# ISU-PAAL/DeepDFA

Hardware: AMD Instinct MI355X
Metric: train_graphs_per_sec (higher is better)
Workload: dtype bf16; 1 GPU; model=DeepDFA-FlowGNN-GGNN(n_steps=5,D=128), global_batch=256, avg_nodes_per_graph=45, parallelism=dp1

## Files before the change

csrc/bindings.hip:

```cpp

#include <torch/extension.h>

#include <hip/hip_runtime.h>
#include <hip/hip_bf16.h>
#include <c10/hip/HIPStream.h>
#include <c10/util/accumulate.h>

#include <climits>

template <typename T>
void launch_embed4_fwd(const T*, const long*, T*, int, int, hipStream_t);
template <typename T, typename TO>
void launch_embed4_fwd2(const T*, const long*, TO*, int, int, hipStream_t);
template <typename T>
void launch_embed4_bwd(const T*, const long*, float*, long, int, hipStream_t);
template <typename T>
void launch_spmm_sum(const int*, const int*, const T*, T*, int, int, hipStream_t);
template <typename T>
void launch_gru_gates_fwd(const T*, const T*, const T*, T*, T*, T*, T*, long, int, hipStream_t);
template <typename T>
void launch_gru_gates_bwd(const T*, const T*, const T*, const T*, const T*, const T*, T*, T*, T*,
                          long, int, hipStream_t);
template <typename T>
void launch_attn_pool_fwd(const T*, const T*, const int*, T*, float*, int, int, hipStream_t);
template <typename T>
void launch_attn_pool_bwd(const T*, const T*, const float*, const int*, T*, T*, float*, int, int,
                          hipStream_t);
void launch_segment_max(const float*, const int*, float*, int, hipStream_t);
template <typename T>
void launch_gru_gates2_fwd(const T*, const T*, T*, T*, T*, T*, T*, long, int, hipStream_t);
template <typename T>
void launch_gru_gates2_bwd(const T*, const T*, const T*, const T*, const T*, const T*, T*, T*,
                           long, int, hipStream_t);
template <typename T>
void launch_colsum(const T*, float*, int, int, hipStream_t);
template <typename T>
void launch_spmm_sum_strided(const int*, const int*, const T*, T*, int, int, long,
                             hipStream_t);
void launch_gemm_bias2(const __hip_bfloat16*, const __hip_bfloat16*, const __hip_bfloat16*,
                       const __hip_bfloat16*, const __hip_bfloat16*, long,
                       const __hip_bfloat16*, long, __hip_bfloat16*, int, int, int, int,
                       hipStream_t);
void launch_gemm_bias(const __hip_bfloat16*, const __hip_bfloat16*, const __hip_bfloat16*,
                      const __hip_bfloat16*, const __hip_bfloat16*, __hip_bfloat16*, int, int,
                      int, int, hipStream_t);
void launch_wgrad(const __hip_bfloat16*, const __hip_bfloat16*, const __hip_bfloat16*, float*,
                  float*, int, int, int, int, hipStream_t, float* = nullptr,
                  float* = nullptr, float* = nullptr, float* = nullptr);
template <typename T>
void launch_layernorm_fwd(const T*, const float*, const float*, T*, float*, float*, long, int,
                          float, hipStream_t);
template <typename T>
void launch_layernorm_bwd(const T*, const T*, const float*, const float*, const float*, T*, long,
                          int, hipStream_t);
template <typename T>
void launch_layernorm_wgrad(const T*, const T*, const float*, const float*, float*, float*, long,
                            int, hipStream_t);
template <typename T>
void launch_bias_gelu_fwd(const T*, const float*, T*, long, int, hipStream_t);
template <typename T>
void launch_bias_gelu_bwd(const T*, const T*, const float*, T*, long, int, hipStream_t);
template <typename T>
void launch_softmax_mask_fwd(const T*, const int*, T*, T*, long, int, int, float, float,
                             unsigned long long, int, int, hipStream_t);
template <typename T>
// ... 264 lines not shown
  CHECK_GPU(B);
  const int K = A.size(0), M = A.size(1), C = B.size(1);
  TORCH_CHECK(B.size(0) == K && M % 64 == 0 && C % 8 == 0);
  const bool acc = out_opt.has_value();
  auto out = acc_or_zeros(out_opt, {M, C}, A.options(), "wgrad");
  if (M % 128 == 0 && C % 128 == 0) {
    launch_wgrad2(ptr<bf16_t>(A), ptr<bf16_t>(B), out.data_ptr<float>(), nullptr,
                  K, M, C, acc ? 1 : 0, cur_stream());
    return out;
  }
  launch_wgrad(ptr<bf16_t>(A), ptr<bf16_t>(B), nullptr, out.data_ptr<float>(), nullptr,
               K, M, C, C, cur_stream());
  return out;
}

void launch_pack_gru_weights(const float*, const float*, const float*, const float*,
                             const float*, const float*, int, __hip_bfloat16*,
                             __hip_bfloat16*, __hip_bfloat16*, __hip_bfloat16*,
                             __hip_bfloat16*, __hip_bfloat16*, __hip_bfloat16*,
                             __hip_bfloat16*, hipStream_t);
void launch_gemm_gru(const __hip_bfloat16*, const __hip_bfloat16*, const __hip_bfloat16*,
                     const __hip_bfloat16*, const __hip_bfloat16*, __hip_bfloat16*,
                     __hip_bfloat16*, __hip_bfloat16*, __hip_bfloat16*, __hip_bfloat16*,
                     int, int, int, int, hipStream_t);

void pack_gru_weights(at::Tensor W_e, at::Tensor b_e, at::Tensor W_ih, at::Tensor W_hh,
                      at::Tensor b_ih, at::Tensor b_hh, at::Tensor w_e16, at::Tensor b_e16,
                      at::Tensor Wcat, at::Tensor WcatT, at::Tensor b_cat, at::Tensor W_eT,
                      at::Tensor Wcat_perm, at::Tensor b_perm) {
  CHECK_GPU(W_e);
  const int H = W_e.size(0);
  TORCH_CHECK(W_e.scalar_type() == at::kFloat && W_ih.scalar_type() == at::kFloat,
              "pack_gru_weights reads fp32 master weights");
  TORCH_CHECK(Wcat.size(0) == 4 * H && Wcat.size(1) == 2 * H);
  launch_pack_gru_weights(W_e.data_ptr<float>(), b_e.data_ptr<float>(),
                          W_ih.data_ptr<float>(), W_hh.data_ptr<float>(),
                          b_ih.data_ptr<float>(), b_hh.data_ptr<float>(), H,
                          mptr<bf16_t>(w_e16), mptr<bf16_t>(b_e16), mptr<bf16_t>(Wcat),
                          mptr<bf16_t>(WcatT), mptr<bf16_t>(b_cat), mptr<bf16_t>(W_eT),
                          mptr<bf16_t>(Wcat_perm), mptr<bf16_t>(b_perm),
                          cur_stream());
}

std::vector<at::Tensor> ggnn_fused_fwd(at::Tensor indptr, at::Tensor indices, at::Tensor x,
                                       at::Tensor W_e, at::Tensor b_e, at::Tensor Wcat_perm,
                                       at::Tensor b_perm, long n_steps) {
  CHECK_GPU(x);
  TORCH_CHECK(x.scalar_type() == at::kBFloat16, "fused GGNN path is bf16");
  const long N = x.size(0);
  const long H = x.size(1);
  TORCH_CHECK(H % 64 == 0 && (4 * H) % 128 == 0, "H must suit the MFMA tile");
  TORCH_CHECK(Wcat_perm.size(0) == 4 * H && Wcat_perm.size(1) == 2 * H &&
              b_perm.numel() == 4 * H,
              "Wcat_perm/b_perm must be prebuilt (ops/flowgnn.py cache)");
  auto stream = cur_stream();
  const long S = n_steps;
  auto opts = x.options();
  auto HH = at::empty({S + 1, N, H}, opts);
  HH.select(0, 0).copy_(x);
  auto M = at::empty({S, N, H}, opts);
  auto R = at::empty({S, N, H}, opts);
  auto Z = at::empty({S, N, H}, opts);
  auto Nn = at::empty({S, N, H}, opts);
  auto HN = at::empty({S, N, H}, opts);
  auto wh = at::empty({N, H}, opts);
  const long NH = N * H;
  for (long s = 0; s < S; ++s) {
    const bf16_t* h = ptr<bf16_t>(HH) + s * NH;
    launch_gemm_bias(h, nullptr, ptr<bf16_t>(W_e), ptr<bf16_t>(b_e), nullptr, mptr<bf16_t>(wh),
                     N, H, H, H, stream);
    bf16_t* m = mptr<bf16_t>(M) + s * NH;
    launch_spmm_sum<bf16_t>(indptr.data_ptr<int>(), indices.data_ptr<int>(), ptr<bf16_t>(wh), m,
                            N, H, stream);
    launch_gemm_gru(m, h, ptr<bf16_t>(Wcat_perm), ptr<bf16_t>(b_perm), h,
                    mptr<bf16_t>(HH) + (s + 1) * NH, mptr<bf16_t>(R) + s * NH,
                    mptr<bf16_t>(Z) + s * NH, mptr<bf16_t>(Nn) + s * NH,
                    mptr<bf16_t>(HN) + s * NH, N, 2 * H, H, H, stream);
  }
  auto h_final = HH.select(0, S);
  return {h_final, HH, M, R, Z, Nn, HN};
}

std::vector<at::Tensor> ggnn_fused_bwd(at::Tensor grad_out, at::Tensor t_indptr,
                                       at::Tensor t_indices, at::Tensor x, at::Tensor W_eT,
                                       at::Tensor WcatT, at::Tensor HH,
                                       at::Tensor M, at::Tensor R, at::Tensor Z, at::Tensor Nn,
                                       at::Tensor HN, long n_steps,
                                       c10::optional<at::Tensor> out_we,
                                       c10::optional<at::Tensor> out_be,
                                       c10::optional<std::vector<at::Tensor>> gru_outs) {
  const long N = x.size(0);
  const long H = x.size(1);
  const long S = n_steps;
  const long NH = N * H;
  auto stream = cur_stream();
  TORCH_CHECK(WcatT.size(0) == 2 * H && WcatT.size(1) == 4 * H && W_eT.size(0) == H,
              "WcatT/W_eT must be prebuilt (ops/flowgnn.py cache)");
  auto opts = x.options();
  auto Ggicat = at::empty({S, N, 4 * H}, opts);
  auto Gwh = at::empty({S, N, H}, opts);
  auto grad_h = grad_out.contiguous().clone();
  auto grad_hd = at::empty({N, H}, opts);
  auto grad_A = at::empty({N, 2 * H}, opts);
  for (long s = S - 1; s >= 0; --s) {
    const bf16_t* h_in = ptr<bf16_t>(HH) + s * NH;
    auto ggic = Ggicat.select(0, s);
    auto gwh = Gwh.select(0, s);
    launch_gru_gates2_bwd<bf16_t>(ptr<bf16_t>(grad_h), h_in, ptr<bf16_t>(R) + s * NH,
                                  ptr<bf16_t>(Z) + s * NH, ptr<bf16_t>(Nn) + s * NH,
                                  ptr<bf16_t>(HN) + s * NH, mptr<bf16_t>(ggic),
                                  mptr<bf16_t>(grad_hd), NH, H, stream);
    launch_gemm_bias(ptr<bf16_t>(ggic), nullptr, ptr<bf16_t>(WcatT), nullptr, nullptr,
                     mptr<bf16_t>(grad_A), N, 4 * H, 4 * H, 2 * H, stream);
    launch_spmm_sum_strided<bf16_t>(t_indptr.data_ptr<int>(), t_indices.data_ptr<int>(),
                                    ptr<bf16_t>(grad_A), mptr<bf16_t>(gwh), N, H,
                                    2 * H, stream);
    launch_gemm_bias2(ptr<bf16_t>(gwh), nullptr, ptr<bf16_t>(W_eT), nullptr,
                      ptr<bf16_t>(grad_hd), H, ptr<bf16_t>(grad_A) + H, 2 * H,
                      mptr<bf16_t>(grad_h), N, H, H, H, stream);
  }
  auto A_g = Ggicat.view({S * N, 4 * H});
  const bool gru_direct = gru_outs.has_value();
  at::Tensor gWcat, cs4;
  if (gru_direct) {
    TORCH_CHECK(gru_outs->size() == 4, "gru_outs = [gW_ih, gW_hh, gb_ih, gb_hh]");
    for (auto& t : *gru_outs)
      TORCH_CHECK(t.is_cuda() && t.scalar_type() == at::kFloat && t.is_contiguous());
    TORCH_CHECK((*gru_outs)[0].numel() == 3 * H * H &&
                (*gru_outs)[1].numel() == 3 * H * H &&
                (*gru_outs)[2].numel() == 3 * H && (*gru_outs)[3].numel() == 3 * H);
  } else {
    gWcat = at::zeros({4 * H, 2 * H}, opts.dtype(at::kFloat));
    cs4 = at::zeros({4 * H}, opts.dtype(at::kFloat));
  }
  if (gru_direct)
    launch_wgrad(ptr<bf16_t>(A_g), ptr<bf16_t>(M), ptr<bf16_t>(HH), nullptr, nullptr,
                 S * N, 4 * H, 2 * H, H, stream, (*gru_outs)[0].data_ptr<float>(),
                 (*gru_outs)[1].data_ptr<float>(), (*gru_outs)[2].data_ptr<float>(),
                 (*gru_outs)[3].data_ptr<float>());
  else
    launch_wgrad(ptr<bf16_t>(A_g), ptr<bf16_t>(M), ptr<bf16_t>(HH), gWcat.data_ptr<float>(),
                 cs4.data_ptr<float>(), S * N, 4 * H, 2 * H, H, stream);
// ... 774 lines not shown
                     v.data_ptr<float>(), p.numel(), (float)lr, (float)beta1, (float)beta2,
                     (float)eps, (float)weight_decay, step.data_ptr<float>(), gc,
                     l2_mode ? 1 : 0, s16, cur_stream());
}

PYBIND11_MODULE(TORCH_EXTENSION_NAME, m) {
  m.doc() = "deepdfa_amd MI355X (gfx950) kernels";
  m.def("embed4_fwd", &embed4_fwd, pybind11::arg("tables"), pybind11::arg("idx"), pybind11::arg("out_bf16") = false);
  m.def("embed4_bwd", &embed4_bwd, pybind11::arg("grad_out"), pybind11::arg("idx"),
        pybind11::arg("V"), pybind11::arg("Demb"),
        pybind11::arg("out") = pybind11::none());
  m.def("spmm_sum", &spmm_sum);
  m.def("gru_gates_fwd", &gru_gates_fwd);
  m.def("gru_gates_bwd", &gru_gates_bwd);
  m.def("attn_pool_fwd", &attn_pool_fwd);
  m.def("attn_pool_bwd", &attn_pool_bwd);
  m.def("segment_max", &segment_max);
  m.def("gemm_bias", &gemm_bias);
  m.def("wgrad", &wgrad, pybind11::arg("A"), pybind11::arg("B"),
        pybind11::arg("out") = pybind11::none());
  m.def("gru_gates2_fwd", &gru_gates2_fwd);
  m.def("gru_gates2_bwd", &gru_gates2_bwd);
  m.def("colsum", &colsum, pybind11::arg("x"), pybind11::arg("out") = pybind11::none());
  m.def("ggnn_fused_fwd", &ggnn_fused_fwd);
  m.def("pack_gru_weights", &pack_gru_weights);
  m.def("bce_logits_fwd", [](at::Tensor logits, at::Tensor labels,
                             c10::optional<at::Tensor> weight,
                             c10::optional<at::Tensor> pos_weight) {
    CHECK_GPU(logits);
    auto out2 = at::empty({2}, logits.options());
    launch_bce_logits_fwd(
        logits.data_ptr<float>(), labels.data_ptr<float>(),
        weight.has_value() ? weight->data_ptr<float>() : nullptr,
        pos_weight.has_value() ? pos_weight->data_ptr<float>() : nullptr,
        out2.data_ptr<float>(), logits.numel(), cur_stream());
    return out2;
  });
  m.def("bce_logits_bwd", [](at::Tensor logits, at::Tensor labels,
                             c10::optional<at::Tensor> weight,
                             c10::optional<at::Tensor> pos_weight,
                             at::Tensor grad, at::Tensor out2) {
    auto dlogits = at::empty_like(logits);
    launch_bce_logits_bwd(
        logits.data_ptr<float>(), labels.data_ptr<float>(),
        weight.has_value() ? weight->data_ptr<float>() : nullptr,
        pos_weight.has_value() ? pos_weight->data_ptr<float>() : nullptr,
        grad.data_ptr<float>(), out2.data_ptr<float>(),
// ... 200 lines not shown
        pybind11::arg("weight_decay"), pybind11::arg("step"),
        pybind11::arg("gclip") = pybind11::none(),
        pybind11::arg("l2_mode") = false,
        pybind11::arg("p16") = pybind11::none());
  m.def("softmax_mask_bwd", &softmax_mask_bwd);
  m.def("node_head_fwd", &node_head_fwd, pybind11::arg("h"), pybind11::arg("fe"),
        pybind11::arg("W1"), pybind11::arg("W2"), pybind11::arg("b1"), pybind11::arg("b2"),
        pybind11::arg("w3"), pybind11::arg("b3"), pybind11::arg("save") = true,
        pybind11::arg("tile_rows") = 0);
  m.def("node_head_bwd", &node_head_bwd, pybind11::arg("dlogits"), pybind11::arg("H1"),
        pybind11::arg("H2"), pybind11::arg("W1T"), pybind11::arg("W2T"), pybind11::arg("w3"),
        pybind11::arg("out_w3") = pybind11::none(), pybind11::arg("out_b3") = pybind11::none(),
        pybind11::arg("tile_rows") = 0);
  m.def("node_head_tile_rows", [](int64_t N, int64_t tile) {
    return node_head_tile_rows((int)N, (int)tile);
  }, pybind11::arg("N"), pybind11::arg("tile_rows") = 0);
  m.def("ggnn_fused_bwd", &ggnn_fused_bwd, pybind11::arg("grad_out"),
        pybind11::arg("t_indptr"), pybind11::arg("t_indices"), pybind11::arg("x"),
        pybind11::arg("W_eT"), pybind11::arg("WcatT"), pybind11::arg("HH"),
        pybind11::arg("M"), pybind11::arg("R"), pybind11::arg("Z"), pybind11::arg("Nn"),
        pybind11::arg("HN"), pybind11::arg("n_steps"),
        pybind11::arg("out_we") = pybind11::none(),
        pybind11::arg("out_be") = pybind11::none(),
        pybind11::arg("gru_outs") = pybind11::none());
}
```

csrc/flowgnn_kernels.hip:

```cpp

#include <hip/hip_runtime.h>
#include <hip/hip_bf16.h>

#include <algorithm>
using std::min;

#define WAVE 64


template <typename T> __device__ __forceinline__ float to_f(T v);
template <> __device__ __forceinline__ float to_f<float>(float v) { return v; }
template <> __device__ __forceinline__ float to_f<__hip_bfloat16>(__hip_bfloat16 v) {
  return __bfloat162float(v);
}

template <typename T> __device__ __forceinline__ T from_f(float v);
template <> __device__ __forceinline__ float from_f<float>(float v) { return v; }
template <> __device__ __forceinline__ __hip_bfloat16 from_f<__hip_bfloat16>(float v) {
  return __float2bfloat16(v);
}

__device__ __forceinline__ float sigmoidf_(float x) { return 1.0f / (1.0f + __expf(-x)); }


template <typename T, typename TO>
__global__ void embed4_fwd_kernel(const T* __restrict__ tables,
                                  const long* __restrict__ idx,
                                  TO* __restrict__ out, int N, int V) {
// ... 155 lines not shown
    n_o[i] = from_f<T>(n);
    hn_o[i] = from_f<T>(hn);
  }
}

template <typename T>
__global__ void gru_gates2_bwd_kernel(const T* __restrict__ grad_h_new,
                                      const T* __restrict__ h,
                                      const T* __restrict__ r_i,
                                      const T* __restrict__ z_i,
                                      const T* __restrict__ n_i,
                                      const T* __restrict__ hn_i,
                                      T* __restrict__ grad_gicat,
                                      T* __restrict__ grad_h, long NH, int H) {
  for (long i = (long)blockIdx.x * blockDim.x + threadIdx.x; i < NH;
       i += (long)gridDim.x * blockDim.x) {
    const long row = i / H;
    const int c = (int)(i - row * H);
    const long b = row * 4 * H + c;
    const float go = to_f(grad_h_new[i]);
    const float r = to_f(r_i[i]), z = to_f(z_i[i]), n = to_f(n_i[i]);
    const float hn = to_f(hn_i[i]);
    const float hv = to_f(h[i]);
    const float dn = go * (1.f - z);
    const float dz = go * (hv - n);
    const float dpn = dn * (1.f - n * n);
    const float dr = dpn * hn;
    const float dpr = dr * r * (1.f - r);
    const float dpz = dz * z * (1.f - z);
    grad_gicat[b] = from_f<T>(dpr);
    grad_gicat[b + H] = from_f<T>(dpz);
    grad_gicat[b + 2 * H] = from_f<T>(dpn);
    grad_gicat[b + 3 * H] = from_f<T>(dpn * r);
    grad_h[i] = from_f<T>(go * z);
  }
}


template <typename T>
__global__ void colsum_kernel(const T* __restrict__ x, float* __restrict__ out,
                              int N, int C, int rows_per_block) {
  const int c = blockIdx.x * blockDim.x + threadIdx.x;
  if (c >= C) return;
  const int r0 = blockIdx.y * rows_per_block;
  const int r1 = min(r0 + rows_per_block, N);
  float a0 = 0.f, a1 = 0.f, a2 = 0.f, a3 = 0.f;
  int r = r0;
  for (; r + 4 <= r1; r += 4) {
    a0 += to_f(x[(long)r * C + c]);
    a1 += to_f(x[(long)(r + 1) * C + c]);
    a2 += to_f(x[(long)(r + 2) * C + c]);
    a3 += to_f(x[(long)(r + 3) * C + c]);
  }
  for (; r < r1; ++r) a0 += to_f(x[(long)r * C + c]);
  atomicAdd(out + c, (a0 + a1) + (a2 + a3));
}

// ... 436 lines not shown
```

csrc/gemm_bias.hip:

```cpp

#include <hip/hip_runtime.h>

#include "mfma_tile.h"

#define BM 64
#define BN TILE_BN

template <int BMT, bool CT = false>
__global__ __launch_bounds__(256) void gemm_bias_kernel(
    const bf16* __restrict__ A1, const bf16* __restrict__ A2,
    const bf16* __restrict__ W, const bf16* __restrict__ bias,
    const bf16* __restrict__ addend, long astride,
    const bf16* __restrict__ addend2, long astride2,
    bf16* __restrict__ out, int N, int K,
    int K1, int COL) {
  extern __shared__ __attribute__((aligned(16))) char smem[];

  const int r0 = blockIdx.x * BMT;
  const int c0 = blockIdx.y * BN;
  const int lane = threadIdx.x & (WAVE - 1);
  const int wid = threadIdx.x >> 6;
  const int wm = wid >> 1;
  const int wn = wid & 1;

  constexpr int MFRAG = BMT / 32;
  f32x4 acc[MFRAG][4] = {};
  tile_regstaged_gemm<BMT, CT>(acc, smem, A1, A2, K1, W, N, K, COL, r0, c0);

#pragma unroll
  for (int m = 0; m < MFRAG; ++m) {
    const int row_base = r0 + wm * (BMT / 2) + m * 16 + (lane >> 4) * 4;
#pragma unroll
    for (int n = 0; n < 4; ++n) {
      const int col = c0 + wn * 64 + n * 16 + (lane & 15);
      if constexpr (CT) {
        if (col >= COL) continue;
      }
      const float b = bias ? __bfloat162float(bias[col]) : 0.0f;
#pragma unroll
      for (int i = 0; i < 4; ++i) {
        const int row = row_base + i;
        if (row < N) {
          float v = acc[m][n][i] + b;
          if (addend) v += __bfloat162float(addend[(long)row * astride + col]);
          if (addend2) v += __bfloat162float(addend2[(long)row * astride2 + col]);
          out[(long)row * COL + col] = __float2bfloat16(v);
        }
      }
    }
  }
}

void launch_gemm_bias2(const bf16* A1, const bf16* A2, const bf16* W,
                       const bf16* bias, const bf16* addend, long astride,
                       const bf16* addend2, long astride2, bf16* out, int N,
                       int K, int K1, int COL, hipStream_t stream) {
  if (COL % BN != 0) {
    const dim3 grid((N + 31) / 32, (COL + BN - 1) / BN);
    const size_t lds = tile_lds_bytes(32);
    hipLaunchKernelGGL((gemm_bias_kernel<32, true>), grid, dim3(256), lds,
                       stream, A1, A2, W, bias, addend, astride, addend2,
                       astride2, out, N, K, K1, COL);
    return;
  }
  const long blocks64 = (long)((N + BM - 1) / BM) * (COL / BN);
  if (blocks64 < 384) {
    const dim3 grid((N + 31) / 32, COL / BN);
    const size_t lds = tile_lds_bytes(32);
    hipLaunchKernelGGL(gemm_bias_kernel<32>, grid, dim3(256), lds, stream, A1,
                       A2, W, bias, addend, astride, addend2, astride2, out, N,
                       K, K1, COL);
  } else {
    const dim3 grid((N + BM - 1) / BM, COL / BN);
    const size_t lds = tile_lds_bytes(BM);
    hipLaunchKernelGGL(gemm_bias_kernel<BM>, grid, dim3(256), lds, stream, A1,
                       A2, W, bias, addend, astride, addend2, astride2, out, N,
                       K, K1, COL);
  }
}

void launch_gemm_bias(const bf16* A1, const bf16* A2, const bf16* W,
                      const bf16* bias, const bf16* addend, bf16* out, int N,
                      int K, int K1, int COL, hipStream_t stream) {
  launch_gemm_bias2(A1, A2, W, bias, addend, COL, nullptr, 0, out, N, K, K1,
                    COL, stream);
}


__device__ __forceinline__ float sigf_(float x) { return 1.f / (1.f + __expf(-x)); }

#define GRU_TS 132

constexpr size_t gru_lds_bytes(int bmt) {
  const size_t pipe = tile_lds_bytes(bmt), gate = bmt * GRU_TS * sizeof(float);
  return pipe > gate ? pipe : gate;
}

template <int BMT>
__global__ __launch_bounds__(256) void gemm_gru_kernel(
    const bf16* __restrict__ A1, const bf16* __restrict__ A2,
    const bf16* __restrict__ Wperm, const bf16* __restrict__ bperm,
    const bf16* __restrict__ h_in, bf16* __restrict__ h_new,
    bf16* __restrict__ R, bf16* __restrict__ Z, bf16* __restrict__ Nn,
    bf16* __restrict__ HN, int N, int K, int K1, int H) {
  extern __shared__ __attribute__((aligned(16))) char smem[];

  const int r0 = blockIdx.x * BMT;
  const int c0 = blockIdx.y * BN;
  const int tid = threadIdx.x;
  const int lane = tid & (WAVE - 1);
  const int wid = tid >> 6;
  const int wm = wid >> 1;
  const int wn = wid & 1;

  constexpr int MFRAG = BMT / 32;
  f32x4 acc[MFRAG][4] = {};
  tile_regstaged_gemm<BMT, false>(acc, smem, A1, A2, K1, Wperm, N, K, 4 * H,
                                  r0, c0);

  float* tile = reinterpret_cast<float*>(smem);
#pragma unroll
  for (int m = 0; m < MFRAG; ++m) {
    const int row = wm * (BMT / 2) + m * 16 + (lane >> 4) * 4;
#pragma unroll
    for (int n = 0; n < 4; ++n) {
      const int col = wn * 64 + n * 16 + (lane & 15);
      const float b = __bfloat162float(bperm[c0 + col]);
#pragma unroll
      for (int i = 0; i < 4; ++i)
        tile[(row + i) * GRU_TS + col] = acc[m][n][i] + b;
    }
  }
  __syncthreads();

  const int j0 = c0 >> 2;
  for (int it = tid; it < BMT * 32; it += 256) {
    const int row = it >> 5;
    const int jj = it & 31;
    const int gr = r0 + row;
    if (gr >= N) continue;
    const f32x4 gse = *reinterpret_cast<const f32x4*>(tile + row * GRU_TS + jj * 4);
    const float r = sigf_(gse[0]);
    const float z = sigf_(gse[1]);
    const float n = tanhf(gse[2] + r * gse[3]);
    const long o = (long)gr * H + j0 + jj;
    const float hv = __bfloat162float(h_in[o]);
    h_new[o] = __float2bfloat16((1.f - z) * n + z * hv);
    R[o] = __float2bfloat16(r);
    Z[o] = __float2bfloat16(z);
    Nn[o] = __float2bfloat16(n);
    HN[o] = __float2bfloat16(gse[3]);
  }
}

void launch_gemm_gru(const bf16* A1, const bf16* A2, const bf16* Wperm,
                     const bf16* bperm, const bf16* h_in, bf16* h_new, bf16* R,
                     bf16* Z, bf16* Nn, bf16* HN, int N, int K, int K1, int H,
                     hipStream_t stream) {
  const int COL = 4 * H;
  const long blocks64 = (long)((N + BM - 1) / BM) * (COL / BN);
  if (blocks64 < 384) {
    const dim3 grid((N + 31) / 32, COL / BN);
    const size_t lds = gru_lds_bytes(32);
    hipLaunchKernelGGL(gemm_gru_kernel<32>, grid, dim3(256), lds, stream, A1,
                       A2, Wperm, bperm, h_in, h_new, R, Z, Nn, HN, N, K, K1, H);
  } else {
    const dim3 grid((N + BM - 1) / BM, COL / BN);
    const size_t lds = gru_lds_bytes(BM);
    hipLaunchKernelGGL(gemm_gru_kernel<BM>, grid, dim3(256), lds, stream, A1,
                       A2, Wperm, bperm, h_in, h_new, R, Z, Nn, HN, N, K, K1, H);
  }
}
```

csrc/mfma_tile.h:

```cpp

#pragma once

#include <hip/hip_runtime.h>
#include <hip/hip_bf16.h>

#define WAVE 64

using bf16 = __hip_bfloat16;
using bf16x8 = __attribute__((ext_vector_type(8))) __bf16;
using f32x4 = __attribute__((ext_vector_type(4))) float;
using uint4v = __attribute__((ext_vector_type(4))) unsigned int;

#define TILE_BN 128
#define TILE_BK 64
#define TILE_ROWB 128

__device__ __forceinline__ int tile_swz_byte(int row, int byte) {
  return byte ^ ((row & 7) << 4);
}
__device__ __forceinline__ int tile_swz(int row, int byte) {
  return row * TILE_ROWB + tile_swz_byte(row, byte);
}


// ... 56 lines not shown
  const int srow = tid >> 3;
  const int soff = (tid & 7) * 16;
#pragma unroll
  for (int p = 0; p < NP; ++p) {
    const int rr = row0 + srow + p * 32;
    if constexpr (CT) {
      r[p] = {};
      if (rr >= row_end) continue;
    }
    r[p] = *reinterpret_cast<const uint4v*>(W + (long)rr * ldw + kk + soff / 2);
  }
}

template <int NP>
__device__ __forceinline__ void tile_regs_store(char* lds, int tid,
                                                const uint4v r[NP]) {
  const int srow = tid >> 3;
  const int soff = (tid & 7) * 16;
#pragma unroll
  for (int p = 0; p < NP; ++p)
    *reinterpret_cast<uint4v*>(lds + tile_swz(srow + p * 32, soff)) = r[p];
}

template <int BMT, bool CT>
__device__ __forceinline__ void tile_regstaged_gemm(
    f32x4 (&acc)[BMT / 32][4], char* smem, const bf16* __restrict__ A1,
    const bf16* __restrict__ A2, int K1, const bf16* __restrict__ W, int N,
    int K, int COL, int r0, int c0) {
  constexpr int NAR = BMT / 32;
  const int tid = threadIdx.x;
  const int lane = tid & (WAVE - 1);
  const int wm = tid >> 7;
  const int wn = (tid >> 6) & 1;
  const int srow = tid >> 3;
  const int soff = (tid & 7) * 16;
  auto load_regs = [&](int kk, uint4v ar[NAR], uint4v br[4]) {
#pragma unroll
    for (int p = 0; p < NAR; ++p) {
      const int gr = r0 + srow + p * 32;
      ar[p] = {};
      if (gr < N) {
        const int gk = kk + soff / 2;
        const bf16* src = (gk < K1) ? (A1 + (long)gr * K1 + gk)
                                    : (A2 + (long)gr * (K - K1) + (gk - K1));
        ar[p] = *reinterpret_cast<const uint4v*>(src);
      }
    }
    tile_w_load<4, CT>(W, K, c0, kk, COL, tid, br);
  };
  auto write_regs = [&](int i, const uint4v ar[NAR], const uint4v br[4]) {
    tile_regs_store<NAR>(tile_abuf<BMT>(smem, i), tid, ar);
    tile_regs_store<4>(tile_bbuf<BMT>(smem, i), tid, br);
  };
  uint4v areg[NAR], breg[4];
  load_regs(0, areg, breg);
  write_regs(0, areg, breg);
  __syncthreads();
  int cur = 0;
  for (int kk = 0; kk < K; kk += TILE_BK) {
    const bool has_next = (kk + TILE_BK) < K;
    if (has_next) load_regs(kk + TILE_BK, areg, breg);
    tile_kstep<false>(acc, tile_abuf<BMT>(smem, cur), wm * (BMT / 2),
                      tile_bbuf<BMT>(smem, cur), wn * 64, lane);
    if (has_next) write_regs(cur ^ 1, areg, breg);
    __syncthreads();
    cur ^= 1;
  }
}

template <int NP>
__device__ __forceinline__ void tile_glds_stage(const bf16* __restrict__ src_base,
                                                long row_stride_elems, int kk,
                                                char* lds, int wid, int lane) {
#pragma unroll
  for (int c4 = 0; c4 < NP; ++c4) {
    const int c = wid * NP + c4;
    const int row = 8 * c + (lane >> 3);
    const int kbyte = (lane & 7) * 16;
    const int src_byte = tile_swz_byte(row, kbyte);
    const bf16* gsrc = src_base + row * row_stride_elems + kk + src_byte / 2;
    __builtin_amdgcn_global_load_lds(
        reinterpret_cast<const unsigned int*>(gsrc),
        reinterpret_cast<unsigned int*>(lds + c * 1024 + (lane & 63) * 16), 16, 0, 0);
  }
}

template <int BMT>
// ... 28 lines not shown
```

setup.py:

```python

import os

from setuptools import setup

os.environ.setdefault("PYTORCH_ROCM_ARCH", "gfx950")

from torch.utils.cpp_extension import BuildExtension, CUDAExtension

HERE = os.path.dirname(os.path.abspath(__file__))

ext = CUDAExtension(
    name="deepdfa_amd._C",
    sources=[
        "csrc/bindings.hip",
        "csrc/flowgnn_kernels.hip",
        "csrc/gemm_bias.hip",
        "csrc/wgrad.hip",
        "csrc/transformer_kernels.hip",
        "csrc/flash_attn.hip",
        "csrc/gemm_bf16.hip",
        "csrc/wgrad2.hip",
        "csrc/adamw.hip",
        "csrc/lmhead_ce.hip",
        "csrc/node_head.hip",
        "csrc/graph_head.hip",
    ],
    depends=["csrc/mfma_tile.h"],
    extra_compile_args={
        "cxx": ["-O3", "-std=c++17"],
        "nvcc": ["-O3", "-std=c++17"],
    },
)

setup(
    name="deepdfa_amd",
    version="0.1.0",
    packages=["deepdfa_amd"],
    ext_modules=[ext],
    cmdclass={"build_ext": BuildExtension.with_options(no_python_abi_suffix=False)},
)
```

Measured before the change: 475,000 graphs/s.

## Fuse neighbor-sum gather into GEMM A-loads and GRU gate backward into GEMM

The GGNN forward no longer runs a separate SpMM. The GRU GEMM kernel gathers and sums neighbor rows of W_e·h while staging its A tiles, and the block with column index 0 writes the aggregated messages out for backward. In backward, a new gates_gemm kernel computes the GRU gate gradients and feeds them straight into the WcatT GEMM, and the transposed SpMM is folded into the following gemm_bias2 A-load. This removes several kernel launches and round trips of intermediate tensors through HBM per step. The cost is irregular gather loads inside the GEMM pipeline, and the gather is repeated for every column block.

After: 494,500 graphs/s (median of 6 runs). +4.1%, better.

```diff
diff --git a/csrc/bindings.hip b/csrc/bindings.hip
--- a/csrc/bindings.hip
+++ b/csrc/bindings.hip
@@ -40,7 +40,12 @@
 void launch_gemm_bias2(const __hip_bfloat16*, const __hip_bfloat16*, const __hip_bfloat16*,
                        const __hip_bfloat16*, const __hip_bfloat16*, long,
                        const __hip_bfloat16*, long, __hip_bfloat16*, int, int, int, int,
-                       hipStream_t);
+                       hipStream_t, const int* = nullptr, const int* = nullptr, long = 0,
+                       __hip_bfloat16* = nullptr);
+bool launch_gates_gemm(const __hip_bfloat16*, const __hip_bfloat16*, const __hip_bfloat16*,
+                       const __hip_bfloat16*, const __hip_bfloat16*, const __hip_bfloat16*,
+                       const __hip_bfloat16*, __hip_bfloat16*, __hip_bfloat16*,
+                       __hip_bfloat16*, int, int, hipStream_t);
 void launch_gemm_bias(const __hip_bfloat16*, const __hip_bfloat16*, const __hip_bfloat16*,
                       const __hip_bfloat16*, const __hip_bfloat16*, __hip_bfloat16*, int, int,
                       int, int, hipStream_t);
@@ -351,7 +356,8 @@
 void launch_gemm_gru(const __hip_bfloat16*, const __hip_bfloat16*, const __hip_bfloat16*,
                      const __hip_bfloat16*, const __hip_bfloat16*, __hip_bfloat16*,
                      __hip_bfloat16*, __hip_bfloat16*, __hip_bfloat16*, __hip_bfloat16*,
-                     int, int, int, int, hipStream_t);
+                     int, int, int, int, hipStream_t, const int* = nullptr,
+                     const int* = nullptr, __hip_bfloat16* = nullptr);
 
 void pack_gru_weights(at::Tensor W_e, at::Tensor b_e, at::Tensor W_ih, at::Tensor W_hh,
                       at::Tensor b_ih, at::Tensor b_hh, at::Tensor w_e16, at::Tensor b_e16,
@@ -373,7 +379,7 @@
 
 std::vector<at::Tensor> ggnn_fused_fwd(at::Tensor indptr, at::Tensor indices, at::Tensor x,
                                        at::Tensor W_e, at::Tensor b_e, at::Tensor Wcat_perm,
-                                       at::Tensor b_perm, long n_steps) {
+                                       at::Tensor b_perm, long n_steps, bool fuse) {
   CHECK_GPU(x);
   TORCH_CHECK(x.scalar_type() == at::kBFloat16, "fused GGNN path is bf16");
   const long N = x.size(0);
@@ -399,12 +405,15 @@
     launch_gemm_bias(h, nullptr, ptr<bf16_t>(W_e), ptr<bf16_t>(b_e), nullptr, mptr<bf16_t>(wh),
                      N, H, H, H, stream);
     bf16_t* m = mptr<bf16_t>(M) + s * NH;
-    launch_spmm_sum<bf16_t>(indptr.data_ptr<int>(), indices.data_ptr<int>(), ptr<bf16_t>(wh), m,
-                            N, H, stream);
-    launch_gemm_gru(m, h, ptr<bf16_t>(Wcat_perm), ptr<bf16_t>(b_perm), h,
-                    mptr<bf16_t>(HH) + (s + 1) * NH, mptr<bf16_t>(R) + s * NH,
+    if (!fuse)
+      launch_spmm_sum<bf16_t>(indptr.data_ptr<int>(), indices.data_ptr<int>(), ptr<bf16_t>(wh),
+                              m, N, H, stream);
+    launch_gemm_gru(fuse ? ptr<bf16_t>(wh) : m, h, ptr<bf16_t>(Wcat_perm), ptr<bf16_t>(b_perm),
+                    h, mptr<bf16_t>(HH) + (s + 1) * NH, mptr<bf16_t>(R) + s * NH,
                     mptr<bf16_t>(Z) + s * NH, mptr<bf16_t>(Nn) + s * NH,
-                    mptr<bf16_t>(HN) + s * NH, N, 2 * H, H, H, stream);
+                    mptr<bf16_t>(HN) + s * NH, N, 2 * H, H, H, stream,
+                    fuse ? indptr.data_ptr<int>() : nullptr,
+                    fuse ? indices.data_ptr<int>() : nullptr, fuse ? m : nullptr);
   }
   auto h_final = HH.select(0, S);
   return {h_final, HH, M, R, Z, Nn, HN};
@@ -417,7 +426,8 @@
                                        at::Tensor HN, long n_steps,
                                        c10::optional<at::Tensor> out_we,
                                        c10::optional<at::Tensor> out_be,
-                                       c10::optional<std::vector<at::Tensor>> gru_outs) {
+                                       c10::optional<std::vector<at::Tensor>> gru_outs,
+                                       bool fuse) {
   const long N = x.size(0);
   const long H = x.size(1);
   const long S = n_steps;
@@ -428,25 +438,41 @@
   auto opts = x.options();
   auto Ggicat = at::empty({S, N, 4 * H}, opts);
   auto Gwh = at::empty({S, N, H}, opts);
-  auto grad_h = grad_out.contiguous().clone();
+  auto go = grad_out.contiguous();
+  auto grad_h = S > 0 ? at::empty({N, H}, opts) : go.clone();
   auto grad_hd = at::empty({N, H}, opts);
   auto grad_A = at::empty({N, 2 * H}, opts);
   for (long s = S - 1; s >= 0; --s) {
     const bf16_t* h_in = ptr<bf16_t>(HH) + s * NH;
+    const bf16_t* g_in = (s == S - 1) ? ptr<bf16_t>(go) : ptr<bf16_t>(grad_h);
     auto ggic = Ggicat.select(0, s);
     auto gwh = Gwh.select(0, s);
-    launch_gru_gates2_bwd<bf16_t>(ptr<bf16_t>(grad_h), h_in, ptr<bf16_t>(R) + s * NH,
-                                  ptr<bf16_t>(Z) + s * NH, ptr<bf16_t>(Nn) + s * NH,
-                                  ptr<bf16_t>(HN) + s * NH, mptr<bf16_t>(ggic),
-                                  mptr<bf16_t>(grad_hd), NH, H, stream);
-    launch_gemm_bias(ptr<bf16_t>(ggic), nullptr, ptr<bf16_t>(WcatT), nullptr, nullptr,
-                     mptr<bf16_t>(grad_A), N, 4 * H, 4 * H, 2 * H, stream);
-    launch_spmm_sum_strided<bf16_t>(t_indptr.data_ptr<int>(), t_indices.data_ptr<int>(),
-                                    ptr<bf16_t>(grad_A), mptr<bf16_t>(gwh), N, H,
-                                    2 * H, stream);
-    launch_gemm_bias2(ptr<bf16_t>(gwh), nullptr, ptr<bf16_t>(W_eT), nullptr,
-                      ptr<bf16_t>(grad_hd), H, ptr<bf16_t>(grad_A) + H, 2 * H,
-                      mptr<bf16_t>(grad_h), N, H, H, H, stream);
+    if (!fuse ||
+        !launch_gates_gemm(g_in, h_in, ptr<bf16_t>(R) + s * NH, ptr<bf16_t>(Z) + s * NH,
+                           ptr<bf16_t>(Nn) + s * NH, ptr<bf16_t>(HN) + s * NH,
+                           ptr<bf16_t>(WcatT), mptr<bf16_t>(ggic), mptr<bf16_t>(grad_hd),
+                           mptr<bf16_t>(grad_A), N, H, stream)) {
+      launch_gru_gates2_bwd<bf16_t>(g_in, h_in, ptr<bf16_t>(R) + s * NH,
+                                    ptr<bf16_t>(Z) + s * NH, ptr<bf16_t>(Nn) + s * NH,
+                                    ptr<bf16_t>(HN) + s * NH, mptr<bf16_t>(ggic),
+                                    mptr<bf16_t>(grad_hd), NH, H, stream);
+      launch_gemm_bias(ptr<bf16_t>(ggic), nullptr, ptr<bf16_t>(WcatT), nullptr, nullptr,
+                       mptr<bf16_t>(grad_A), N, 4 * H, 4 * H, 2 * H, stream);
+    }
+    if (fuse) {
+      launch_gemm_bias2(ptr<bf16_t>(grad_A), nullptr, ptr<bf16_t>(W_eT), nullptr,
+                        ptr<bf16_t>(grad_hd), H, ptr<bf16_t>(grad_A) + H, 2 * H,
+                        mptr<bf16_t>(grad_h), N, H, H, H, stream,
+                        t_indptr.data_ptr<int>(), t_indices.data_ptr<int>(), 2 * H,
+                        mptr<bf16_t>(gwh));
+    } else {
+      launch_spmm_sum_strided<bf16_t>(t_indptr.data_ptr<int>(), t_indices.data_ptr<int>(),
+                                      ptr<bf16_t>(grad_A), mptr<bf16_t>(gwh), N, H,
+                                      2 * H, stream);
+      launch_gemm_bias2(ptr<bf16_t>(gwh), nullptr, ptr<bf16_t>(W_eT), nullptr,
+                        ptr<bf16_t>(grad_hd), H, ptr<bf16_t>(grad_A) + H, 2 * H,
+                        mptr<bf16_t>(grad_h), N, H, H, H, stream);
+    }
   }
   auto A_g = Ggicat.view({S * N, 4 * H});
   const bool gru_direct = gru_outs.has_value();
@@ -1267,7 +1293,10 @@
   m.def("gru_gates2_fwd", &gru_gates2_fwd);
   m.def("gru_gates2_bwd", &gru_gates2_bwd);
   m.def("colsum", &colsum, pybind11::arg("x"), pybind11::arg("out") = pybind11::none());
-  m.def("ggnn_fused_fwd", &ggnn_fused_fwd);
+  m.def("ggnn_fused_fwd", &ggnn_fused_fwd, pybind11::arg("indptr"), pybind11::arg("indices"),
+        pybind11::arg("x"), pybind11::arg("W_e"), pybind11::arg("b_e"),
+        pybind11::arg("Wcat_perm"), pybind11::arg("b_perm"), pybind11::arg("n_steps"),
+        pybind11::arg("fuse") = true);
   m.def("pack_gru_weights", &pack_gru_weights);
   m.def("bce_logits_fwd", [](at::Tensor logits, at::Tensor labels,
                              c10::optional<at::Tensor> weight,
@@ -1514,5 +1543,5 @@
         pybind11::arg("HN"), pybind11::arg("n_steps"),
         pybind11::arg("out_we") = pybind11::none(),
         pybind11::arg("out_be") = pybind11::none(),
-        pybind11::arg("gru_outs") = pybind11::none());
-}
+        pybind11::arg("gru_outs") = pybind11::none(), pybind11::arg("fuse") = true);
+}
diff --git a/csrc/flowgnn_kernels.hip b/csrc/flowgnn_kernels.hip
--- a/csrc/flowgnn_kernels.hip
+++ b/csrc/flowgnn_kernels.hip
@@ -4,6 +4,8 @@
 
 #include <algorithm>
 using std::min;
+
+#include "gru_gate_bwd.h"
 
 #define WAVE 64
 
@@ -205,17 +207,12 @@
     const float r = to_f(r_i[i]), z = to_f(z_i[i]), n = to_f(n_i[i]);
     const float hn = to_f(hn_i[i]);
     const float hv = to_f(h[i]);
-    const float dn = go * (1.f - z);
-    const float dz = go * (hv - n);
-    const float dpn = dn * (1.f - n * n);
-    const float dr = dpn * hn;
-    const float dpr = dr * r * (1.f - r);
-    const float dpz = dz * z * (1.f - z);
-    grad_gicat[b] = from_f<T>(dpr);
-    grad_gicat[b + H] = from_f<T>(dpz);
-    grad_gicat[b + 2 * H] = from_f<T>(dpn);
-    grad_gicat[b + 3 * H] = from_f<T>(dpn * r);
-    grad_h[i] = from_f<T>(go * z);
+    const GruGate2Grad d = gru_gate2_bwd_elem(go, hv, r, z, n, hn);
+    grad_gicat[b] = from_f<T>(d.dpr);
+    grad_gicat[b + H] = from_f<T>(d.dpz);
+    grad_gicat[b + 2 * H] = from_f<T>(d.dpn);
+    grad_gicat[b + 3 * H] = from_f<T>(d.dpnr);
+    grad_h[i] = from_f<T>(d.ghd);
   }
 }
 
diff --git a/csrc/gemm_bias.hip b/csrc/gemm_bias.hip
--- a/csrc/gemm_bias.hip
+++ b/csrc/gemm_bias.hip
@@ -6,29 +6,16 @@
 #define BM 64
 #define BN TILE_BN
 
-template <int BMT, bool CT = false>
-__global__ __launch_bounds__(256) void gemm_bias_kernel(
-    const bf16* __restrict__ A1, const bf16* __restrict__ A2,
-    const bf16* __restrict__ W, const bf16* __restrict__ bias,
+constexpr int gather_gpf(int bmt) { return bmt == 32 ? 4 : 2; }
+
+template <int BMT, bool CT>
+__device__ __forceinline__ void gemm_bias_epilogue(
+    const f32x4 (&acc)[BMT / 32][4], const bf16* __restrict__ bias,
     const bf16* __restrict__ addend, long astride,
-    const bf16* __restrict__ addend2, long astride2,
-    bf16* __restrict__ out, int N, int K,
-    int K1, int COL) {
-  extern __shared__ __attribute__((aligned(16))) char smem[];
-
-  const int r0 = blockIdx.x * BMT;
-  const int c0 = blockIdx.y * BN;
-  const int lane = threadIdx.x & (WAVE - 1);
-  const int wid = threadIdx.x >> 6;
-  const int wm = wid >> 1;
-  const int wn = wid & 1;
-
-  constexpr int MFRAG = BMT / 32;
-  f32x4 acc[MFRAG][4] = {};
-  tile_regstaged_gemm<BMT, CT>(acc, smem, A1, A2, K1, W, N, K, COL, r0, c0);
-
-#pragma unroll
-  for (int m = 0; m < MFRAG; ++m) {
+    const bf16* __restrict__ addend2, long astride2, bf16* __restrict__ out,
+    int N, int COL, int r0, int c0, int lane, int wm, int wn) {
+#pragma unroll
+  for (int m = 0; m < BMT / 32; ++m) {
     const int row_base = r0 + wm * (BMT / 2) + m * 16 + (lane >> 4) * 4;
 #pragma unroll
     for (int n = 0; n < 4; ++n) {
@@ -51,31 +38,76 @@
   }
 }
 
+template <int BMT, bool CT = false, int GPF = 0>
+__global__ __launch_bounds__(256) void gemm_bias_kernel(
+    const bf16* __restrict__ A1, const bf16* __restrict__ A2,
+    const bf16* __restrict__ W, const bf16* __restrict__ bias,
+    const bf16* __restrict__ addend, long astride,
+    const bf16* __restrict__ addend2, long astride2,
+    bf16* __restrict__ out, int N, int K,
+    int K1, int COL, TileGather g) {
+  extern __shared__ __attribute__((aligned(16))) char smem[];
+
+  const int r0 = blockIdx.x * BMT;
+  const int c0 = blockIdx.y * BN;
+  const int lane = threadIdx.x & (WAVE - 1);
+  const int wid = threadIdx.x >> 6;
+  const int wm = wid >> 1;
+  const int wn = wid & 1;
+
+  constexpr int MFRAG = BMT / 32;
+  f32x4 acc[MFRAG][4] = {};
+  if (blockIdx.y != 0) g.out = nullptr;
+  tile_regstaged_gemm<BMT, CT, GPF>(acc, smem, A1, A2, K1, W, N, K, COL, r0,
+                                       c0, g);
+  gemm_bias_epilogue<BMT, CT>(acc, bias, addend, astride, addend2, astride2,
+                              out, N, COL, r0, c0, lane, wm, wn);
+}
+
 void launch_gemm_bias2(const bf16* A1, const bf16* A2, const bf16* W,
                        const bf16* bias, const bf16* addend, long astride,
                        const bf16* addend2, long astride2, bf16* out, int N,
-                       int K, int K1, int COL, hipStream_t stream) {
+                       int K, int K1, int COL, hipStream_t stream,
+                       const int* g_indptr, const int* g_indices, long g_lda,
+                       bf16* g_out) {
+  const bool g = g_indptr != nullptr;
+  const TileGather tg = {g_indptr, g_indices, g_lda, g_out};
   if (COL % BN != 0) {
     const dim3 grid((N + 31) / 32, (COL + BN - 1) / BN);
     const size_t lds = tile_lds_bytes(32);
-    hipLaunchKernelGGL((gemm_bias_kernel<32, true>), grid, dim3(256), lds,
-                       stream, A1, A2, W, bias, addend, astride, addend2,
-                       astride2, out, N, K, K1, COL);
+    if (g)
+      hipLaunchKernelGGL((gemm_bias_kernel<32, true, gather_gpf(32)>), grid, dim3(256),
+                         lds, stream, A1, A2, W, bias, addend, astride, addend2,
+                         astride2, out, N, K, K1, COL, tg);
+    else
+      hipLaunchKernelGGL((gemm_bias_kernel<32, true>), grid, dim3(256), lds,
+                         stream, A1, A2, W, bias, addend, astride, addend2,
+                         astride2, out, N, K, K1, COL, tg);
     return;
   }
   const long blocks64 = (long)((N + BM - 1) / BM) * (COL / BN);
   if (blocks64 < 384) {
     const dim3 grid((N + 31) / 32, COL / BN);
     const size_t lds = tile_lds_bytes(32);
-    hipLaunchKernelGGL(gemm_bias_kernel<32>, grid, dim3(256), lds, stream, A1,
-                       A2, W, bias, addend, astride, addend2, astride2, out, N,
-                       K, K1, COL);
+    if (g)
+      hipLaunchKernelGGL((gemm_bias_kernel<32, false, gather_gpf(32)>), grid, dim3(256),
+                         lds, stream, A1, A2, W, bias, addend, astride, addend2,
+                         astride2, out, N, K, K1, COL, tg);
+    else
+      hipLaunchKernelGGL(gemm_bias_kernel<32>, grid, dim3(256), lds, stream,
+                         A1, A2, W, bias, addend, astride, addend2, astride2,
+                         out, N, K, K1, COL, tg);
   } else {
     const dim3 grid((N + BM - 1) / BM, COL / BN);
     const size_t lds = tile_lds_bytes(BM);
-    hipLaunchKernelGGL(gemm_bias_kernel<BM>, grid, dim3(256), lds, stream, A1,
-                       A2, W, bias, addend, astride, addend2, astride2, out, N,
-                       K, K1, COL);
+    if (g)
+      hipLaunchKernelGGL((gemm_bias_kernel<BM, false, gather_gpf(BM)>), grid, dim3(256),
+                         lds, stream, A1, A2, W, bias, addend, astride, addend2,
+                         astride2, out, N, K, K1, COL, tg);
+    else
+      hipLaunchKernelGGL(gemm_bias_kernel<BM>, grid, dim3(256), lds, stream,
+                         A1, A2, W, bias, addend, astride, addend2, astride2,
+                         out, N, K, K1, COL, tg);
   }
 }
 
@@ -83,7 +115,7 @@
                       const bf16* bias, const bf16* addend, bf16* out, int N,
                       int K, int K1, int COL, hipStream_t stream) {
   launch_gemm_bias2(A1, A2, W, bias, addend, COL, nullptr, 0, out, N, K, K1,
-                    COL, stream);
+                    COL, stream, nullptr, nullptr, 0, nullptr);
 }
 
 
@@ -96,13 +128,13 @@
   return pipe > gate ? pipe : gate;
 }
 
-template <int BMT>
+template <int BMT, int GPF = 0>
 __global__ __launch_bounds__(256) void gemm_gru_kernel(
     const bf16* __restrict__ A1, const bf16* __restrict__ A2,
     const bf16* __restrict__ Wperm, const bf16* __restrict__ bperm,
     const bf16* __restrict__ h_in, bf16* __restrict__ h_new,
     bf16* __restrict__ R, bf16* __restrict__ Z, bf16* __restrict__ Nn,
-    bf16* __restrict__ HN, int N, int K, int K1, int H) {
+    bf16* __restrict__ HN, int N, int K, int K1, int H, TileGather g) {
   extern __shared__ __attribute__((aligned(16))) char smem[];
 
   const int r0 = blockIdx.x * BMT;
@@ -115,8 +147,9 @@
 
   constexpr int MFRAG = BMT / 32;
   f32x4 acc[MFRAG][4] = {};
-  tile_regstaged_gemm<BMT, false>(acc, smem, A1, A2, K1, Wperm, N, K, 4 * H,
-                                  r0, c0);
+  if (blockIdx.y != 0) g.out = nullptr;
+  tile_regstaged_gemm<BMT, false, GPF>(acc, smem, A1, A2, K1, Wperm, N, K,
+                                          4 * H, r0, c0, g);
 
   float* tile = reinterpret_cast<float*>(smem);
 #pragma unroll
@@ -156,18 +189,171 @@
 void launch_gemm_gru(const bf16* A1, const bf16* A2, const bf16* Wperm,
                      const bf16* bperm, const bf16* h_in, bf16* h_new, bf16* R,
                      bf16* Z, bf16* Nn, bf16* HN, int N, int K, int K1, int H,
-                     hipStream_t stream) {
+                     hipStream_t stream, const int* g_indptr,
+                     const int* g_indices, bf16* g_out) {
   const int COL = 4 * H;
+  const bool g = g_indptr != nullptr;
+  const TileGather tg = {g_indptr, g_indices, (long)K1, g_out};
   const long blocks64 = (long)((N + BM - 1) / BM) * (COL / BN);
   if (blocks64 < 384) {
     const dim3 grid((N + 31) / 32, COL / BN);
     const size_t lds = gru_lds_bytes(32);
-    hipLaunchKernelGGL(gemm_gru_kernel<32>, grid, dim3(256), lds, stream, A1,
-                       A2, Wperm, bperm, h_in, h_new, R, Z, Nn, HN, N, K, K1, H);
+    if (g)
+      hipLaunchKernelGGL((gemm_gru_kernel<32, gather_gpf(32)>), grid, dim3(256), lds,
+                         stream, A1, A2, Wperm, bperm, h_in, h_new, R, Z, Nn,
+                         HN, N, K, K1, H, tg);
+    else
+      hipLaunchKernelGGL(gemm_gru_kernel<32>, grid, dim3(256), lds, stream, A1,
+                         A2, Wperm, bperm, h_in, h_new, R, Z, Nn, HN, N, K, K1,
+                         H, tg);
   } else {
     const dim3 grid((N + BM - 1) / BM, COL / BN);
     const size_t lds = gru_lds_bytes(BM);
-    hipLaunchKernelGGL(gemm_gru_kernel<BM>, grid, dim3(256), lds, stream, A1,
-                       A2, Wperm, bperm, h_in, h_new, R, Z, Nn, HN, N, K, K1, H);
-  }
-}
+    if (g)
+      hipLaunchKernelGGL((gemm_gru_kernel<BM, gather_gpf(BM)>), grid, dim3(256), lds,
+                         stream, A1, A2, Wperm, bperm, h_in, h_new, R, Z, Nn,
+                         HN, N, K, K1, H, tg);
+    else
+      hipLaunchKernelGGL(gemm_gru_kernel<BM>, grid, dim3(256), lds, stream, A1,
+                         A2, Wperm, bperm, h_in, h_new, R, Z, Nn, HN, N, K, K1,
+                         H, tg);
+  }
+}
+
+
+#include "gru_gate_bwd.h"
+
+#define GG_WBUF (TILE_BN * TILE_ROWB)
+#define GG_PF 3
+
+template <int BMT, int NSL>
+__global__ __launch_bounds__(256) void gates_gemm_kernel(
+    const bf16* __restrict__ grad_h, const bf16* __restrict__ h_in,
+    const bf16* __restrict__ R, const bf16* __restrict__ Z,
+    const bf16* __restrict__ Nn, const bf16* __restrict__ HN,
+    const bf16* __restrict__ WcatT, bf16* __restrict__ ggic_out,
+    bf16* __restrict__ grad_hd, bf16* __restrict__ grad_A, int N) {
+  constexpr int H = NSL * 16;
+  constexpr int K = 4 * H;
+  constexpr int COL = 2 * H;
+  constexpr int HC = H / 8;
+  constexpr int SPG = NSL / 4;
+  __shared__ __attribute__((aligned(16))) char smem[BMT * NSL * TILE_ROWB + 2 * GG_WBUF];
+  char* act = smem;
+  char* wbuf = smem + BMT * NSL * TILE_ROWB;
+
+  const int r0 = blockIdx.x * BMT;
+  const int c0 = blockIdx.y * BN;
+  const int tid = threadIdx.x;
+  const int lane = tid & (WAVE - 1);
+  const int wid = tid >> 6;
+  const int wm = wid >> 1;
+  const int wn = wid & 1;
+  const bool save = blockIdx.y == 0;
+
+  uint4v wr[GG_PF][4];
+#pragma unroll
+  for (int t = 0; t < GG_PF; ++t)
+    tile_w_load<4>(WcatT, K, c0, t * TILE_BK, COL, tid, wr[t]);
+
+  constexpr int NIT = BMT * HC / 256;
+  static_assert(BMT * HC % 256 == 0, "whole items per thread");
+#pragma unroll
+  for (int q = 0; q < NIT; ++q) {
+    const int it = tid + q * 256;
+    const int row = it / HC;
+    const int c = it % HC;
+    const int gr = r0 + row;
+    tile_pack8 o[4];
+#pragma unroll
+    for (int g = 0; g < 4; ++g) o[g].v = uint4v{0u, 0u, 0u, 0u};
+    if (gr < N) {
+      const long off = (long)gr * H + c * 8;
+      tile_pack8 go, hv, r, z, n, hn, hd;
+      go.v = *reinterpret_cast<const uint4v*>(grad_h + off);
+      hv.v = *reinterpret_cast<const uint4v*>(h_in + off);
+      r.v = *reinterpret_cast<const uint4v*>(R + off);
+      z.v = *reinterpret_cast<const uint4v*>(Z + off);
+      n.v = *reinterpret_cast<const uint4v*>(Nn + off);
+      hn.v = *reinterpret_cast<const uint4v*>(HN + off);
+#pragma unroll
+      for (int j = 0; j < 8; ++j) {
+        const GruGate2Grad d = gru_gate2_bwd_elem(
+            __bfloat162float(go.e[j]), __bfloat162float(hv.e[j]),
+            __bfloat162float(r.e[j]), __bfloat162float(z.e[j]),
+            __bfloat162float(n.e[j]), __bfloat162float(hn.e[j]));
+        o[0].e[j] = __float2bfloat16(d.dpr);
+        o[1].e[j] = __float2bfloat16(d.dpz);
+        o[2].e[j] = __float2bfloat16(d.dpn);
+        o[3].e[j] = __float2bfloat16(d.dpnr);
+        hd.e[j] = __float2bfloat16(d.ghd);
+      }
+      if (save) {
+#pragma unroll
+        for (int g = 0; g < 4; ++g)
+          *reinterpret_cast<uint4v*>(ggic_out + (long)gr * K + g * H + c * 8) = o[g].v;
+        *reinterpret_cast<uint4v*>(grad_hd + off) = hd.v;
+      }
+    }
+#pragma unroll
+    for (int g = 0; g < 4; ++g)
+      *reinterpret_cast<uint4v*>(act + (g * SPG + (c >> 3)) * BMT * TILE_ROWB +
+                                 tile_swz(row, (c & 7) * 16)) = o[g].v;
+  }
+  tile_regs_store<4>(wbuf, tid, wr[0]);
+  if (GG_PF < NSL) tile_w_load<4>(WcatT, K, c0, GG_PF * TILE_BK, COL, tid, wr[0]);
+  __syncthreads();
+
+  constexpr int MFRAG = BMT / 32;
+  f32x4 acc[MFRAG][4] = {};
+#pragma unroll
+  for (int s = 0; s < NSL; ++s) {
+    const int cur = s & 1;
+    tile_kstep<false>(acc, act + s * BMT * TILE_ROWB, wm * (BMT / 2),
+                      wbuf + cur * GG_WBUF, wn * 64, lane);
+    if (s + 1 < NSL)
+      tile_regs_store<4>(wbuf + (cur ^ 1) * GG_WBUF, tid, wr[(s + 1) % GG_PF]);
+    if (s + 1 + GG_PF < NSL)
+      tile_w_load<4>(WcatT, K, c0, (s + 1 + GG_PF) * TILE_BK, COL, tid,
+                     wr[(s + 1) % GG_PF]);
+    __syncthreads();
+  }
+  gemm_bias_epilogue<BMT, false>(acc, nullptr, nullptr, 0, nullptr, 0, grad_A,
+                                 N, COL, r0, c0, lane, wm, wn);
+}
+
+template <int BMT, int NSL>
+static void gates_gemm_launch(const bf16* grad_h, const bf16* h_in,
+                              const bf16* R, const bf16* Z, const bf16* Nn,
+                              const bf16* HN, const bf16* WcatT, bf16* ggic,
+                              bf16* grad_hd, bf16* grad_A, int N,
+                              hipStream_t stream) {
+  const dim3 grid((N + BMT - 1) / BMT, NSL * 32 / BN);
+  hipLaunchKernelGGL((gates_gemm_kernel<BMT, NSL>), grid, dim3(256), 0, stream,
+                     grad_h, h_in, R, Z, Nn, HN, WcatT, ggic, grad_hd, grad_A,
+                     N);
+}
+
+bool launch_gates_gemm(const bf16* grad_h, const bf16* h_in, const bf16* R,
+                       const bf16* Z, const bf16* Nn, const bf16* HN,
+                       const bf16* WcatT, bf16* ggic, bf16* grad_hd,
+                       bf16* grad_A, int N, int H, hipStream_t stream) {
+  if (H != 64 && H != 128 && H != 192) return false;
+  if (N <= 0) return true;
+  const long blocks64 = (long)((N + BM - 1) / BM) * (2 * H / BN);
+  const bool small = blocks64 < 384;
+#define GG_CASE(h)                                                            \
+  if (H == h) {                                                               \
+    if (small)                                                                \
+      gates_gemm_launch<32, h / 16>(grad_h, h_in, R, Z, Nn, HN, WcatT, ggic,  \
+                                    grad_hd, grad_A, N, stream);              \
+    else                                                                      \
+      gates_gemm_launch<BM, h / 16>(grad_h, h_in, R, Z, Nn, HN, WcatT, ggic,  \
+                                    grad_hd, grad_A, N, stream);              \
+  }
+  GG_CASE(64)
+  GG_CASE(128)
+  GG_CASE(192)
+#undef GG_CASE
+  return true;
+}
diff --git a/csrc/gru_gate_bwd.h b/csrc/gru_gate_bwd.h
--- /dev/null
+++ b/csrc/gru_gate_bwd.h
@@ -0,0 +1,20 @@
+
+#pragma once
+
+#include <hip/hip_runtime.h>
+
+struct GruGate2Grad {
+  float dpr, dpz, dpn, dpnr, ghd;
+};
+
+__device__ __forceinline__ GruGate2Grad gru_gate2_bwd_elem(float go, float hv,
+                                                           float r, float z,
+                                                           float n, float hn) {
+  const float dn = go * (1.f - z);
+  const float dz = go * (hv - n);
+  const float dpn = dn * (1.f - n * n);
+  const float dr = dpn * hn;
+  const float dpr = dr * r * (1.f - r);
+  const float dpz = dz * z * (1.f - z);
+  return {dpr, dpz, dpn, dpn * r, go * z};
+}
diff --git a/csrc/mfma_tile.h b/csrc/mfma_tile.h
--- a/csrc/mfma_tile.h
+++ b/csrc/mfma_tile.h
@@ -102,25 +102,106 @@
     *reinterpret_cast<uint4v*>(lds + tile_swz(srow + p * 32, soff)) = r[p];
 }
 
-template <int BMT, bool CT>
+struct TileGather {
+  const int* indptr;
+  const int* indices;
+  long lda;
+  bf16* out;
+};
+
+union tile_pack8 {
+  uint4v v;
+  bf16 e[8];
+};
+
+template <int GPF>
+__device__ __forceinline__ uint4v tile_gather_finish(const uint4v raw[GPF],
+                                                     const bf16* __restrict__ src,
+                                                     long lda,
+                                                     const int* __restrict__ indices,
+                                                     int e0, int e1) {
+  float a[8] = {0.f, 0.f, 0.f, 0.f, 0.f, 0.f, 0.f, 0.f};
+  tile_pack8 v0, v1;
+#pragma unroll
+  for (int q = 0; q < GPF; ++q) {
+    if (e0 + q < e1) {
+      v0.v = raw[q];
+#pragma unroll
+      for (int j = 0; j < 8; ++j) a[j] += __bfloat162float(v0.e[j]);
+    }
+  }
+  for (int e = e0 + GPF; e < e1; e += 2) {
+    const bool two = e + 1 < e1;
+    const int i0 = indices[e];
+    const int i1 = indices[two ? e + 1 : e];
+    v0.v = *reinterpret_cast<const uint4v*>(src + (long)i0 * lda);
+    v1.v = *reinterpret_cast<const uint4v*>(src + (long)i1 * lda);
+#pragma unroll
+    for (int j = 0; j < 8; ++j) a[j] += __bfloat162float(v0.e[j]);
+    if (two) {
+#pragma unroll
+      for (int j = 0; j < 8; ++j) a[j] += __bfloat162float(v1.e[j]);
+    }
+  }
+  tile_pack8 o;
+#pragma unroll
+  for (int j = 0; j < 8; ++j) o.e[j] = __float2bfloat16(a[j]);
+  return o.v;
+}
+
+template <int BMT, bool CT, int GPF = 0>
 __device__ __forceinline__ void tile_regstaged_gemm(
     f32x4 (&acc)[BMT / 32][4], char* smem, const bf16* __restrict__ A1,
     const bf16* __restrict__ A2, int K1, const bf16* __restrict__ W, int N,
-    int K, int COL, int r0, int c0) {
+    int K, int COL, int r0, int c0, const TileGather g = {}) {
   constexpr int NAR = BMT / 32;
+  constexpr bool GATHER = GPF > 0;
+  constexpr int NPF = GATHER ? GPF : 1;
   const int tid = threadIdx.x;
   const int lane = tid & (WAVE - 1);
   const int wm = tid >> 7;
   const int wn = (tid >> 6) & 1;
   const int srow = tid >> 3;
   const int soff = (tid & 7) * 16;
-  auto load_regs = [&](int kk, uint4v ar[NAR], uint4v br[4]) {
+  int ge0[NAR], ge1[NAR], gi[NAR][NPF];
+  if constexpr (GATHER) {
+#pragma unroll
+    for (int p = 0; p < NAR; ++p) {
+      const int gr = r0 + srow + p * 32;
+      ge0[p] = ge1[p] = 0;
+      if (gr < N) {
+        ge0[p] = g.indptr[gr];
+        ge1[p] = g.indptr[gr + 1];
+      }
+    }
+#pragma unroll
+    for (int p = 0; p < NAR; ++p)
+#pragma unroll
+      for (int q = 0; q < NPF; ++q) {
+        gi[p][q] = 0;
+        if (ge0[p] + q < ge1[p]) gi[p][q] = g.indices[ge0[p] + q];
+      }
+  }
+  auto load_regs = [&](int kk, uint4v ar[NAR], uint4v araw[NAR][NPF],
+                       uint4v br[4]) {
+    const int gk = kk + soff / 2;
 #pragma unroll
     for (int p = 0; p < NAR; ++p) {
       const int gr = r0 + srow + p * 32;
       ar[p] = {};
+      if constexpr (GATHER) {
+        if (kk < K1) {
+#pragma unroll
+          for (int q = 0; q < NPF; ++q) {
+            araw[p][q] = {};
+            if (ge0[p] + q < ge1[p])
+              araw[p][q] = *reinterpret_cast<const uint4v*>(
+                  A1 + (long)gi[p][q] * g.lda + gk);
+          }
+          continue;
+        }
+      }
       if (gr < N) {
-        const int gk = kk + soff / 2;
         const bf16* src = (gk < K1) ? (A1 + (long)gr * K1 + gk)
                                     : (A2 + (long)gr * (K - K1) + (gk - K1));
         ar[p] = *reinterpret_cast<const uint4v*>(src);
@@ -128,21 +209,35 @@
     }
     tile_w_load<4, CT>(W, K, c0, kk, COL, tid, br);
   };
-  auto write_regs = [&](int i, const uint4v ar[NAR], const uint4v br[4]) {
+  auto write_regs = [&](int i, int kk, uint4v ar[NAR],
+                        const uint4v araw[NAR][NPF], const uint4v br[4]) {
+    if constexpr (GATHER) {
+      if (kk < K1) {
+        const int gk = kk + soff / 2;
+#pragma unroll
+        for (int p = 0; p < NAR; ++p) {
+          const int gr = r0 + srow + p * 32;
+          ar[p] = tile_gather_finish<NPF>(araw[p], A1 + gk, g.lda, g.indices, ge0[p],
+                                     ge1[p]);
+          if (g.out && gr < N)
+            *reinterpret_cast<uint4v*>(g.out + (long)gr * K1 + gk) = ar[p];
+        }
+      }
+    }
     tile_regs_store<NAR>(tile_abuf<BMT>(smem, i), tid, ar);
     tile_regs_store<4>(tile_bbuf<BMT>(smem, i), tid, br);
   };
-  uint4v areg[NAR], breg[4];
-  load_regs(0, areg, breg);
-  write_regs(0, areg, breg);
+  uint4v areg[NAR], areg2[NAR][NPF], breg[4];
+  load_regs(0, areg, areg2, breg);
+  write_regs(0, 0, areg, areg2, breg);
   __syncthreads();
   int cur = 0;
   for (int kk = 0; kk < K; kk += TILE_BK) {
     const bool has_next = (kk + TILE_BK) < K;
-    if (has_next) load_regs(kk + TILE_BK, areg, breg);
+    if (has_next) load_regs(kk + TILE_BK, areg, areg2, breg);
     tile_kstep<false>(acc, tile_abuf<BMT>(smem, cur), wm * (BMT / 2),
                       tile_bbuf<BMT>(smem, cur), wn * 64, lane);
-    if (has_next) write_regs(cur ^ 1, areg, breg);
+    if (has_next) write_regs(cur ^ 1, kk + TILE_BK, areg, areg2, breg);
     __syncthreads();
     cur ^= 1;
   }
diff --git a/setup.py b/setup.py
--- a/setup.py
+++ b/setup.py
@@ -25,7 +25,7 @@
         "csrc/node_head.hip",
         "csrc/graph_head.hip",
     ],
-    depends=["csrc/mfma_tile.h"],
+    depends=["csrc/mfma_tile.h", "csrc/gru_gate_bwd.h"],
     extra_compile_args={
         "cxx": ["-O3", "-std=c++17"],
         "nvcc": ["-O3", "-std=c++17"],
```
